# smacke/ffsubsync

Hardware: NVIDIA H100
Metric: alignments/sec (2h@100Hz signals) (higher is better)
Workload: dtype int64 VAD; f32 FFT nomination + f64 exact re-score

## Files before the change

### __graft_entry__.py

```python
import os
import subprocess
import sys

ROOT = os.path.dirname(os.path.abspath(__file__))
CSRC = os.path.join(ROOT, "ffsubsync_b200", "csrc")
LIB_DIR = os.path.join(ROOT, "ffsubsync_b200", "_lib")
LIB = os.path.join(LIB_DIR, "libffsubsync_b200.so")
EMUL = os.path.join(ROOT, "tests", "host_emul", "corr_emul")
EMUL_BIG = os.path.join(ROOT, "tests", "host_emul", "bigfft_emul")
EMUL_VAD = os.path.join(ROOT, "tests", "host_emul", "vad_emul")
EMUL_RUNS = os.path.join(ROOT, "tests", "host_emul", "runcorr_emul")

NVCC_FLAGS = [
    "-gencode", "arch=compute_90a,code=sm_90a", "-lineinfo", "-O3", "-std=c++17",
    "-Xcompiler", "-fPIC", "-Xcompiler", "-ffp-contract=off", "--fmad=true", "--extended-lambda",
    "-Wno-deprecated-gpu-targets",
]


def _sources():
    return sorted(os.path.join(CSRC, f) for f in os.listdir(CSRC) if f.endswith(".cu"))


def _stale(target, deps):
    if not os.path.exists(target):
        return True
    t = os.path.getmtime(target)
    return any(os.path.getmtime(d) > t for d in deps)


def build(force: bool = False, verbose: bool = False) -> None:
    nvcc = os.environ.get("NVCC", "/usr/local/cuda/bin/nvcc")
    os.makedirs(LIB_DIR, exist_ok=True)
    srcs = _sources()
    hdrs = [os.path.join(CSRC, f) for f in os.listdir(CSRC) if f.endswith((".cuh", ".h"))]
    hdrs.append(os.path.join(ROOT, "include", "ffsubsync_b200.h"))
    if force or _stale(LIB, srcs + hdrs):
        objs = []
        for s in srcs:
            o = os.path.join(LIB_DIR, os.path.basename(s)[:-3] + ".o")
            if force or _stale(o, [s] + hdrs):
                cmd = [nvcc] + NVCC_FLAGS + (["-Xptxas", "-v"] if verbose else []) + ["-c", s, "-o", o]
                subprocess.check_call(cmd)
            objs.append(o)
        subprocess.check_call([nvcc, "-shared", "-o", LIB] + objs + ["-Wno-deprecated-gpu-targets"])
    emu_src = EMUL + ".cu"
    if os.path.exists(emu_src) and (force or _stale(EMUL, [emu_src, os.path.join(CSRC, "corr.cuh")])):
        subprocess.check_call([nvcc, "-O2", "-std=c++17", "-Wno-deprecated-gpu-targets", "-o", EMUL, emu_src])
    big_src = EMUL_BIG + ".cu"
    if os.path.exists(big_src) and (force or _stale(EMUL_BIG, [big_src, os.path.join(CSRC, "corr.cuh"),
                                                               os.path.join(CSRC, "bigfft.cuh")])):
        subprocess.check_call([nvcc, "-O2", "-std=c++17", "--extended-lambda", "-Wno-deprecated-gpu-targets",
                               "-o", EMUL_BIG, big_src])
    runs_src = EMUL_RUNS + ".cu"
    if os.path.exists(runs_src) and (force or _stale(EMUL_RUNS, [runs_src, os.path.join(CSRC, "runcorr.cuh")])):
        subprocess.check_call([nvcc, "-O2", "-std=c++17", "-Wno-deprecated-gpu-targets", "-o", EMUL_RUNS, runs_src])
    vad_src = EMUL_VAD + ".cu"
    if os.path.exists(vad_src) and (force or _stale(EMUL_VAD, [vad_src, os.path.join(CSRC, "vad_lane.cuh"),
                                                               os.path.join(CSRC, "vad_group.cuh")])):
        subprocess.check_call([nvcc, "-O2", "-std=c++17", "-gencode", "arch=compute_90a,code=sm_90a",
                               "-Wno-deprecated-gpu-targets", "-o", EMUL_VAD, vad_src])
    sys.path.insert(0, ROOT)
    import ffsubsync_b200
    from ffsubsync_b200 import _native

    _native.load()


def smoke() -> None:
    sys.path.insert(0, ROOT)
    import numpy as np

    from ffsubsync_b200.aligners import FFTAligner, MaxScoreAligner
    from ffsubsync_b200.speech_transformers import _make_auditok_detector, _make_energy_zcr_detector
    from oracle import aligner_oracle as ao
    from oracle import auditok_oracle as au
    from oracle import vad_oracle as vo

    rng = np.random.RandomState(0)
    cls = (rng.rand(2000) > 0.5).astype(np.uint8)
    pcm = vo.synth_pcm(cls, 160, seed=1)
    got = _make_energy_zcr_detector(100, 16000, 0.0)(pcm.tobytes())
    want = vo.energy_zcr_detect(pcm.tobytes(), 100, 16000, 0.0)
    assert np.array_equal(got, want), "VAD mismatch"
    got_a = _make_auditok_detector(100, 16000, 0.0)(pcm.tobytes())
    assert np.array_equal(got_a, au.auditok_detect_fast(pcm.tobytes(), 100, 16000, 0.0)), "auditok mismatch"
    ref = want
    sub = np.concatenate([np.zeros(123), ref])[: len(ref)]
    score, off = FFTAligner(max_offset_samples=600).fit_transform(ref, sub, get_score=True)
    wscore, woff = ao.fft_align(ref, sub, 600)
    assert off == woff == -123, (off, woff)
    assert abs(score - wscore) <= 1e-5 * abs(wscore), (score, wscore)
    (s2, o2), _ = MaxScoreAligner(FFTAligner, None, 100, 6).fit_transform(ref, [sub, sub[::-1].copy()])
    assert o2 == -123
    print("smoke ok: vad windows=%d offset=%d score=%.1f" % (len(got), off, score))


if __name__ == "__main__":
    build(force="--force" in sys.argv, verbose="-v" in sys.argv)
    if "--smoke" in sys.argv:
        smoke()
```

### ffsubsync_b200/csrc/runcorr.cu

```cuda
#include <limits.h>
#include <math.h>

#include <algorithm>

#include "common.cuh"
#include "corr_jobs.cuh"
#include "runcorr.cuh"

namespace {

using namespace runcorr;
static_assert(kMaxWindow == kRunMaxWindow, "run path window bound");

struct RunRef {
  long long ref_off;
  long long q_off;
  int R;
};

struct RunStat {
  double mx;
  double eps;
  int total;
  int arg;
};

__device__ __forceinline__ int block_excl_scan(int v, int* sh, int* total) {
  const int lane = threadIdx.x & 31, warp = threadIdx.x >> 5, nw = blockDim.x >> 5;
  int x = v;
#pragma unroll
  for (int d = 1; d < 32; d <<= 1) {
    const int y = __shfl_up_sync(0xffffffffu, x, d);
    if (lane >= d) x += y;
  }
  if (lane == 31) sh[warp] = x;
  __syncthreads();
  if (warp == 0) {
    int s = lane < nw ? sh[lane] : 0;
    const int own = s;
#pragma unroll
    for (int d = 1; d < 32; d <<= 1) {
      const int y = __shfl_up_sync(0xffffffffu, s, d);
      if (lane >= d) s += y;
    }
    sh[lane] = s - own;
    if (lane == 31) sh[32] = s;
  }
  __syncthreads();
  const int r = sh[warp] + x - v;
  *total = sh[32];
  __syncthreads();
  return r;
}

__global__ void __launch_bounds__(1024) ref_bits_kernel(const float* __restrict__ ref, const RunRef* __restrict__ vids,
                                                        uint2* __restrict__ q_all) {
  __shared__ int sh[33];
  const RunRef v = vids[blockIdx.x];
  const float* r = ref + v.ref_off;
  uint2* q = q_all + v.q_off;
  const int lane = threadIdx.x & 31, warp = threadIdx.x >> 5;
  const int n_words = (v.R >> 5) + 2;
  if (threadIdx.x == 0) q[0] = make_uint2(0u, 0u);
  int carry = 0;
  for (int w0 = 0; w0 < n_words; w0 += blockDim.x) {
    const int wb = w0 + 32 * warp;
    float x[32];
#pragma unroll
    for (int u = 0; u < 32; ++u) {
      const long long i = 32LL * (wb + u) + lane;
      x[u] = i < v.R ? __ldg(r + i) : 0.f;
    }
    uint32_t mine = 0;
#pragma unroll
    for (int u = 0; u < 32; ++u) {
      const long long i = 32LL * (wb + u) + lane;
      const uint32_t bal = __ballot_sync(0xffffffffu, i < v.R && x[u] == 1.0f);
      if (lane == u) mine = bal;
    }
    const int w = wb + lane;
    int tot;
    const int ex = block_excl_scan(__popc(mine), sh, &tot);
    if (w < n_words) q[w + 1] = make_uint2(mine, (uint32_t)(carry + ex));
    carry += tot;
  }
}

__global__ void __launch_bounds__(kMaxThreads) run_corr_kernel(const SelJob* __restrict__ sel,
                                                                const long long* __restrict__ job_q,
                                                                const uint2* __restrict__ q_all,
                                                                const uint32_t* __restrict__ sub_bits,
                                                                float ref_label, int max_runs,
                                                                RunStat* __restrict__ stat,
                                                                int* __restrict__ cand_off) {
  extern __shared__ int rsm[];
  int* ra = rsm;
  int* rb = ra + max_runs;
  int* rl = rb + max_runs;
  __shared__ int sh[33];
  __shared__ double smx[32];
  __shared__ int sarg[32];
  const int j = blockIdx.x, tid = threadIdx.x, nthr = blockDim.x;
  const SelJob job = sel[j];
  if (job.kind != 0 || job.m_lo > job.m_hi) {
    if (tid == 0) stat[j] = RunStat{-INFINITY, 0.0, 0, 0};
    return;
  }
  const int R = job.R, S = job.S;
  const uint32_t* bits = sub_bits + job.bits_off;
  const int nws = S >> 5;
  int n_end = 0;
  for (int w0 = 0; w0 <= nws; w0 += nthr) {
    const int w = w0 + tid;
    uint32_t t = 0;
    if (w <= nws) {
      const int nb = S - 32 * w;
      const uint32_t x = nb >= 32 ? __ldg(bits + w) : (nb > 0 ? __ldg(bits + w) & ((1u << nb) - 1u) : 0u);
      const uint32_t prev = w > 0 ? __ldg(bits + w - 1) : 0u;
      t = x ^ ((x << 1) | (prev >> 31));
    }
    int tot;
    int idx = n_end + block_excl_scan(__popc(t), sh, &tot);
    while (t) {
      const int e = 32 * w + __ffs(t) - 1;
      t &= t - 1;
      if (idx < 2 * max_runs) (idx & 1 ? rb : ra)[idx >> 1] = e;
      ++idx;
    }
    n_end += tot;
  }
  const int nr = min(n_end >> 1, max_runs);
  __syncthreads();
  for (int r0 = 0, carry = 0; r0 < nr; r0 += nthr) {
    const int r = r0 + tid;
    const int len = r < nr ? rb[r] - ra[r] : 0;
    int tot;
    const int ex = block_excl_scan(len, sh, &tot);
    if (r < nr) rl[r] = carry + ex;
    carry += tot;
  }
  __syncthreads();
  const uint2* q = q_all + job_q[j];
  const int o_lo = job.o_first + job.m_lo, o_hi = job.o_first + job.m_hi;
  const int o0 = o_lo + kOffsetsPerThread * tid;
  const int n_mine = o0 <= o_hi ? min(kOffsetsPerThread, o_hi - o0 + 1) : 0;
  const RcLevels lv = rc_levels(job.sub_level, ref_label);
  int cnt[32], base = 0;
  if (n_mine > 0) {
    rc_thread_counts(q, R, ra, rb, nr, o0, cnt, base);
  } else {
#pragma unroll
    for (int t = 0; t < 32; ++t) cnt[t] = 0;
  }
  double best = -INFINITY;
  int barg = INT_MIN;
  {
    int um = base;
#pragma unroll
    for (int i = 0; i < 32; ++i) {
      if (i < n_mine) {
        const double g = rc_score(q, R, S, ra, rb, rl, nr, o0 + i, um, lv);
        if (g >= best) {
          best = g;
          barg = o0 + i;
        }
      }
      um += cnt[i] - nr;
    }
  }
  for (int d = 16; d > 0; d >>= 1) {
    const double ob = __shfl_xor_sync(0xffffffffu, best, d);
    const int oa = __shfl_xor_sync(0xffffffffu, barg, d);
    if (ob > best || (ob == best && oa > barg)) {
      best = ob;
      barg = oa;
    }
  }
  if ((tid & 31) == 0) {
    smx[tid >> 5] = best;
    sarg[tid >> 5] = barg;
  }
  __syncthreads();
  double mx = smx[0];
  int arg = sarg[0];
  for (int w = 1; w < (nthr >> 5); ++w)
    if (smx[w] > mx || (smx[w] == mx && sarg[w] > arg)) {
      mx = smx[w];
      arg = sarg[w];
    }
  const double eps = rc_eps((double)min(R, S), lv);
  const double cut = mx - eps;
  uint32_t hit = 0;
  {
    int um = base;
#pragma unroll
    for (int i = 0; i < 32; ++i) {
      if (i < n_mine && rc_score(q, R, S, ra, rb, rl, nr, o0 + i, um, lv) >= cut) hit |= 1u << i;
      um += cnt[i] - nr;
    }
  }
  int total;
  const int h = __popc(hit);
  int rank = block_excl_scan(h, sh, &total);
  rank = total - rank - h;
  while (hit && rank < kCandMax) {
    const int i = 31 - __clz(hit);
    hit &= ~(1u << i);
    cand_off[(size_t)j * kCandMax + rank] = o0 + i;
    ++rank;
  }
  if (tid == 0) stat[j] = RunStat{mx, eps, total, arg};
}

__global__ void __launch_bounds__(128) run_finalize_kernel(const SelJob* __restrict__ sel, int n_jobs, int K,
                                                            int winner_only, const RunStat* __restrict__ stat,
                                                            B2CandBuffers cb) {
  const int j = blockIdx.x * blockDim.x + threadIdx.x;
  if (j >= n_jobs) return;
  const SelJob job = sel[j];
  if (job.kind != 0 || job.m_lo > job.m_hi) {
    cb.cand_cnt[j] = 0;
    cb.job_stat[j] = make_float2(-INFINITY, 0.f);
    return;
  }
  const RunStat st = stat[j];
  cb.job_stat[j] = make_float2((float)st.mx, (float)st.eps);
  if (winner_only && !job.no_prune) {
    const int b0 = (j / K) * K;
    double best_floor = -INFINITY;
    for (int k = 0; k < K; ++k) {
      const RunStat s = stat[b0 + k];
      best_floor = fmax(best_floor, s.mx - s.eps);
    }
    if (fmax(st.mx, (double)(float)st.mx) + st.eps < best_floor) {
      cb.cand_off[(size_t)j * kCandMax] = st.arg;
      cb.cand_cnt[j] = -1;
      return;
    }
  }
  cb.cand_cnt[j] = st.total;
  const int n = min(st.total, kCandMax);
  const int slot = atomicAdd(cb.work_count, n);
  for (int i = 0; i < n; ++i) cb.work_list[slot + i] = (j << 5) | i;
}

}

int b2i_align_runs(b2_ctx* h, const float* d_ref, const int64_t* ref_off, int V, const int* trk_off, int K,
                   std::vector<SelJob>& sel, const uint32_t* d_bits, int max_runs, float ref_label, int winner_only,
                   const B2CandBuffers& cb, const SelJob** d_sel_out) {
  B2Range range("b2:align runs (ref_bits, run_corr, finalize)");
  const size_t J = sel.size();
  std::vector<RunRef> vids;
  std::vector<long long> job_q(J, 0);
  long long q_total = 0;
  int max_thr = 32;
  for (int v = 0; v < V; ++v) {
    const int R = (int)(ref_off[v + 1] - ref_off[v]);
    bool any = false;
    for (size_t j = (size_t)trk_off[v] * K; j < (size_t)trk_off[v + 1] * K; ++j) {
      SelJob& s = sel[j];
      if (s.kind != 0) continue;
      const long long w = (long long)s.m_hi - s.m_lo + 1;
      s.o_first = s.m_lo;
      s.m_lo = 0;
      s.m_hi = (int)(w - 1);
      max_thr = std::max<int>(max_thr, (int)(32 * ceil_div64(ceil_div64(w, kOffsetsPerThread), 32)));
      job_q[j] = q_total;
      any = true;
    }
    if (!any) continue;
    vids.push_back(RunRef{(long long)ref_off[v], q_total, R});
    q_total += rc_ref_entries(R);
  }
  if (max_thr > kMaxThreads) B2_FAIL(h, B2_ERR_UNSUPPORTED, "align runs: window wider than %d offsets", kMaxWindow);
  void* d_ws;
  const size_t q_bytes = ((size_t)q_total * 8 + 15) & ~size_t(15);
  B2_TRY(b2i_ws(h, b2_ctx::WS_RUNS, q_bytes + J * sizeof(RunStat) + 64, &d_ws));
  uint2* q = (uint2*)d_ws;
  RunStat* stat = (RunStat*)((char*)d_ws + q_bytes);
  MetaArena a;
  B2_TRY(b2i_meta_begin(h, &a, J * sizeof(SelJob) + J * 8 + vids.size() * sizeof(RunRef) + 256));
  const SelJob* d_sel = (const SelJob*)b2i_meta_put(&a, sel.data(), J * sizeof(SelJob));
  const long long* d_job_q = (const long long*)b2i_meta_put(&a, job_q.data(), J * 8);
  const RunRef* d_vids = vids.empty() ? nullptr : (const RunRef*)b2i_meta_put(&a, vids.data(), vids.size() * sizeof(RunRef));
  B2_TRY(b2i_meta_commit(&a));
  *d_sel_out = d_sel;
  if (!vids.empty()) {
    ref_bits_kernel<<<(unsigned)vids.size(), 1024, 0, h->stream>>>(d_ref, d_vids, q);
    B2_CHECK_LAUNCH(h, "ref_bits_kernel");
  }
  max_runs = std::max(1, max_runs);
  const size_t smem = (size_t)3 * max_runs * sizeof(int);
  B2_CUDA(h, cudaFuncSetAttribute(run_corr_kernel, cudaFuncAttributeMaxDynamicSharedMemorySize, (int)smem));
  run_corr_kernel<<<(unsigned)J, (unsigned)max_thr, smem, h->stream>>>(d_sel, d_job_q, q, d_bits, ref_label, max_runs,
                                                                      stat, cb.cand_off);
  B2_CHECK_LAUNCH(h, "run_corr_kernel");
  B2_CUDA(h, cudaMemsetAsync(cb.work_count, 0, sizeof(int), h->stream));
  run_finalize_kernel<<<(unsigned)((J + 127) / 128), 128, 0, h->stream>>>(d_sel, (int)J, K, winner_only, stat, cb);
  B2_CHECK_LAUNCH(h, "run_finalize_kernel");
  return B2_OK;
}
```

### ffsubsync_b200/csrc/runcorr.cuh

```cuda
#pragma once
#include <math.h>
#include <stdint.h>

#include <cuda_runtime.h>

#ifdef __CUDACC__
#define RC_HD __host__ __device__ __forceinline__
#else
#define RC_HD inline
#endif

namespace runcorr {

constexpr int kOffsetsPerThread = 32;
constexpr int kMaxThreads = 1024;
constexpr int kMaxWindow = kOffsetsPerThread * kMaxThreads;
constexpr int kRunsPerFlush = 7;

RC_HD uint32_t rc_funnel_r(uint32_t lo, uint32_t hi, int s) {
#ifdef __CUDA_ARCH__
  return __funnelshift_r(lo, hi, (unsigned)s);
#else
  return s == 0 ? lo : (lo >> s) | (hi << (32 - s));
#endif
}

RC_HD int rc_popc(uint32_t x) {
#ifdef __CUDA_ARCH__
  return __popc(x);
#else
  return __builtin_popcount(x);
#endif
}

RC_HD uint2 rc_load(const uint2* p) {
#ifdef __CUDA_ARCH__
  return __ldg(p);
#else
  return *p;
#endif
}

RC_HD long long rc_ref_entries(int R) { return (long long)(R >> 5) + 3; }

RC_HD void rc_ref_window(const uint2* q, int R, int p, uint32_t& win, int& pre) {
  p = p < -32 ? -32 : (p > R ? R : p);
  const int w = p >> 5, s = p & 31;
  const uint2 a = rc_load(q + w + 1), b = rc_load(q + w + 2);
  win = rc_funnel_r(a.x, b.x, s);
  pre = (int)a.y + rc_popc(a.x & ((1u << s) - 1u));
}

RC_HD int rc_ref_prefix(const uint2* q, int R, int p) {
  uint32_t w;
  int pre;
  rc_ref_window(q, R, p, w, pre);
  return pre;
}

RC_HD void rc_flush(uint32_t (&nib)[4], int (&cnt)[32]) {
#pragma unroll
  for (int k = 0; k < 4; ++k) {
#pragma unroll
    for (int i = 0; i < 8; ++i) cnt[4 * i + k] += (int)((nib[k] >> (4 * i)) & 15u);
    nib[k] = 0;
  }
}

RC_HD void rc_thread_counts(const uint2* q, int R, const int* ra, const int* rb, int nr, int o0, int (&cnt)[32],
                            int& base) {
#pragma unroll
  for (int t = 0; t < 32; ++t) cnt[t] = 0;
  uint32_t nib[4] = {0u, 0u, 0u, 0u};
  base = 0;
  int r = 0;
  while (r < nr) {
    const int r_end = nr - r < kRunsPerFlush ? nr : r + kRunsPerFlush;
    for (; r < r_end; ++r) {
      const int a = ra[r], b = rb[r];
      uint32_t wa, wb;
      int pa, pb;
      rc_ref_window(q, R, a + o0, wa, pa);
      rc_ref_window(q, R, b + o0, wb, pb);
      base += pb - pa;
      wa = ~wa;
#pragma unroll
      for (int k = 0; k < 4; ++k) nib[k] += ((wb >> k) & 0x11111111u) + ((wa >> k) & 0x11111111u);
    }
    rc_flush(nib, cnt);
  }
}

RC_HD int rc_sub_prefix(const int* ra, const int* rb, const int* rc, int nr, int x) {
  int lo = 0, hi = nr;
  while (lo < hi) {
    const int mid = (lo + hi) >> 1;
    if (ra[mid] < x) lo = mid + 1;
    else hi = mid;
  }
  if (lo == 0) return 0;
  const int e = rb[lo - 1] < x ? rb[lo - 1] : x;
  return rc[lo - 1] + e - ra[lo - 1];
}

struct RcLevels {
  double hi, alpha, hia;
};

RC_HD RcLevels rc_levels(float sub_level, float ref_label) {
  RcLevels l;
  l.hi = 2.0 * (double)sub_level - 1.0;
  l.alpha = 2.0 * (double)ref_label - 1.0;
  l.hia = l.hi * l.alpha;
  return l;
}

RC_HD double rc_score(const uint2* q, int R, int S, const int* ra, const int* rb, const int* rc, int nr, int o,
                      int um, const RcLevels& l) {
  const int j_lo = o < 0 ? -o : 0;
  const int j_hi = S < R - o ? S : R - o;
  if (j_hi <= j_lo) return 0.0;
  const int n_ov = j_hi - j_lo;
  const int mw = rc_ref_prefix(q, R, j_hi + o) - rc_ref_prefix(q, R, j_lo + o);
  const int uo = rc_sub_prefix(ra, rb, rc, nr, j_hi) - rc_sub_prefix(ra, rb, rc, nr, j_lo);
  const double c11 = um, c01 = mw - um, c10 = uo - um, c00 = n_ov - mw - uo + um;
  return (l.hi * c11 - c01) + (l.hia * c10 - l.alpha * c00);
}

RC_HD double rc_eps(double n, const RcLevels& l) {
  const double u = 1.1102230246251565e-16;
  const double ah = fabs(l.hi), aa = fabs(l.alpha);
  const double c = (ah > 1.0 ? ah : 1.0) * (aa > 1.0 ? aa : 1.0);
  const double k = n + 32.0;
  const double gamma = k * u / (1.0 - k * u);
  return 2.02 * (gamma + 8.0 * u) * n * c;
}

}
```

Baseline: 12460.

## Stage reference bit words in shared memory and incrementalize run-correlation scoring

Splits ref_bits_kernel into chunked blocks plus a separate prefix-fixup kernel so each video's bit-packing runs in parallel across many blocks instead of one serial block. In run_corr_kernel, reference words touched by run endpoints are staged cooperatively into shared memory spans, and per-offset counts use hierarchical nibble/byte/halfword packed accumulators. Per-offset scores now come from a precomputed window scan built with popcounts, replacing repeated binary searches and global loads. The hit pass is skipped for threads whose best score is below the cut, and a 512-thread variant with register caps is added. The cost is extra shared memory, an extra kernel launch, and more complex indexing.

```diff
diff --git a/__graft_entry__.py b/__graft_entry__.py
--- a/__graft_entry__.py
+++ b/__graft_entry__.py
@@ -10,6 +10,7 @@
 EMUL_BIG = os.path.join(ROOT, "tests", "host_emul", "bigfft_emul")
 EMUL_VAD = os.path.join(ROOT, "tests", "host_emul", "vad_emul")
 EMUL_RUNS = os.path.join(ROOT, "tests", "host_emul", "runcorr_emul")
+EMUL_STAGE = os.path.join(ROOT, "tests", "host_emul", "runcorr_stage_emul")
 
 NVCC_FLAGS = [
     "-gencode", "arch=compute_90a,code=sm_90a", "-lineinfo", "-O3", "-std=c++17",
@@ -55,6 +56,9 @@
     runs_src = EMUL_RUNS + ".cu"
     if os.path.exists(runs_src) and (force or _stale(EMUL_RUNS, [runs_src, os.path.join(CSRC, "runcorr.cuh")])):
         subprocess.check_call([nvcc, "-O2", "-std=c++17", "-Wno-deprecated-gpu-targets", "-o", EMUL_RUNS, runs_src])
+    stage_src = EMUL_STAGE + ".cu"
+    if os.path.exists(stage_src) and (force or _stale(EMUL_STAGE, [stage_src, os.path.join(CSRC, "runcorr.cuh")])):
+        subprocess.check_call([nvcc, "-O2", "-std=c++17", "-Wno-deprecated-gpu-targets", "-o", EMUL_STAGE, stage_src])
     vad_src = EMUL_VAD + ".cu"
     if os.path.exists(vad_src) and (force or _stale(EMUL_VAD, [vad_src, os.path.join(CSRC, "vad_lane.cuh"),
                                                                os.path.join(CSRC, "vad_group.cuh")])):
diff --git a/ffsubsync_b200/csrc/runcorr.cu b/ffsubsync_b200/csrc/runcorr.cu
--- a/ffsubsync_b200/csrc/runcorr.cu
+++ b/ffsubsync_b200/csrc/runcorr.cu
@@ -16,6 +16,7 @@
   long long ref_off;
   long long q_off;
   int R;
+  int tot_off;
 };
 
 struct RunStat {
@@ -25,6 +26,8 @@
   int arg;
 };
 
+constexpr int kRefChunkWords = 1024;
+
 __device__ __forceinline__ int block_excl_scan(int v, int* sh, int* total) {
   const int lane = threadIdx.x & 31, warp = threadIdx.x >> 5, nw = blockDim.x >> 5;
   int x = v;
@@ -54,49 +57,70 @@
 }
 
 __global__ void __launch_bounds__(1024) ref_bits_kernel(const float* __restrict__ ref, const RunRef* __restrict__ vids,
-                                                        uint2* __restrict__ q_all) {
+                                                        uint2* __restrict__ q_all, int* __restrict__ chunk_tot) {
   __shared__ int sh[33];
-  const RunRef v = vids[blockIdx.x];
+  const RunRef v = vids[blockIdx.y];
+  const int n_words = (v.R >> 5) + 2;
+  const int w0 = blockIdx.x * kRefChunkWords;
+  if (w0 >= n_words) return;
   const float* r = ref + v.ref_off;
   uint2* q = q_all + v.q_off;
   const int lane = threadIdx.x & 31, warp = threadIdx.x >> 5;
+  if (blockIdx.x == 0 && threadIdx.x == 0) q[0] = make_uint2(0u, 0u);
+  const int wb = w0 + 32 * warp;
+  float x[32];
+#pragma unroll
+  for (int u = 0; u < 32; ++u) {
+    const long long i = 32LL * (wb + u) + lane;
+    x[u] = i < v.R ? __ldg(r + i) : 0.f;
+  }
+  uint32_t mine = 0;
+#pragma unroll
+  for (int u = 0; u < 32; ++u) {
+    const long long i = 32LL * (wb + u) + lane;
+    const uint32_t bal = __ballot_sync(0xffffffffu, i < v.R && x[u] == 1.0f);
+    if (lane == u) mine = bal;
+  }
+  const int w = wb + lane;
+  int tot;
+  const int ex = block_excl_scan(__popc(mine), sh, &tot);
+  if (w < n_words) q[w + 1] = make_uint2(mine, (uint32_t)ex);
+  if (threadIdx.x == 0) chunk_tot[v.tot_off + blockIdx.x] = tot;
+}
+
+__global__ void __launch_bounds__(256) ref_prefix_kernel(const RunRef* __restrict__ vids, uint2* __restrict__ q_all,
+                                                         const int* __restrict__ chunk_tot) {
+  __shared__ int sh[8];
+  const RunRef v = vids[blockIdx.y];
   const int n_words = (v.R >> 5) + 2;
-  if (threadIdx.x == 0) q[0] = make_uint2(0u, 0u);
-  int carry = 0;
-  for (int w0 = 0; w0 < n_words; w0 += blockDim.x) {
-    const int wb = w0 + 32 * warp;
-    float x[32];
-#pragma unroll
-    for (int u = 0; u < 32; ++u) {
-      const long long i = 32LL * (wb + u) + lane;
-      x[u] = i < v.R ? __ldg(r + i) : 0.f;
-    }
-    uint32_t mine = 0;
-#pragma unroll
-    for (int u = 0; u < 32; ++u) {
-      const long long i = 32LL * (wb + u) + lane;
-      const uint32_t bal = __ballot_sync(0xffffffffu, i < v.R && x[u] == 1.0f);
-      if (lane == u) mine = bal;
-    }
-    const int w = wb + lane;
-    int tot;
-    const int ex = block_excl_scan(__popc(mine), sh, &tot);
-    if (w < n_words) q[w + 1] = make_uint2(mine, (uint32_t)(carry + ex));
-    carry += tot;
-  }
-}
-
-__global__ void __launch_bounds__(kMaxThreads) run_corr_kernel(const SelJob* __restrict__ sel,
-                                                                const long long* __restrict__ job_q,
-                                                                const uint2* __restrict__ q_all,
-                                                                const uint32_t* __restrict__ sub_bits,
-                                                                float ref_label, int max_runs,
-                                                                RunStat* __restrict__ stat,
-                                                                int* __restrict__ cand_off) {
+  const int c = blockIdx.x, w0 = c * kRefChunkWords;
+  if (c == 0 || w0 >= n_words) return;
+  int s = 0;
+  for (int i = threadIdx.x; i < c; i += blockDim.x) s += chunk_tot[v.tot_off + i];
+#pragma unroll
+  for (int d = 16; d > 0; d >>= 1) s += __shfl_xor_sync(0xffffffffu, s, d);
+  if ((threadIdx.x & 31) == 0) sh[threadIdx.x >> 5] = s;
+  __syncthreads();
+  s = 0;
+  for (int k = 0; k < (int)(blockDim.x >> 5); ++k) s += sh[k];
+  uint2* q = q_all + v.q_off;
+  const int w1 = min(n_words, w0 + kRefChunkWords);
+  for (int w = w0 + (int)threadIdx.x; w < w1; w += blockDim.x) q[w + 1].y += (uint32_t)s;
+}
+
+template <int kThreads>
+__global__ void __launch_bounds__(kThreads) __maxnreg__(kThreads == kSmallThreads ? 80 : 64) run_corr_kernel(const SelJob* __restrict__ sel,
+                                                             const long long* __restrict__ job_q,
+                                                             const uint2* __restrict__ q_all,
+                                                             const uint32_t* __restrict__ sub_bits,
+                                                             float ref_label, int max_runs,
+                                                             RunStat* __restrict__ stat,
+                                                             int* __restrict__ cand_off) {
   extern __shared__ int rsm[];
-  int* ra = rsm;
-  int* rb = ra + max_runs;
-  int* rl = rb + max_runs;
+  int* ends = rsm;
+  int* rl = ends + 2 * max_runs;
+  uint32_t* sb = (uint32_t*)(rl + max_runs);
+  uint32_t* sp = sb + kStageWords;
   __shared__ int sh[33];
   __shared__ double smx[32];
   __shared__ int sarg[32];
@@ -124,7 +148,7 @@
     while (t) {
       const int e = 32 * w + __ffs(t) - 1;
       t &= t - 1;
-      if (idx < 2 * max_runs) (idx & 1 ? rb : ra)[idx >> 1] = e;
+      if (idx < 2 * max_runs) ends[idx] = e;
       ++idx;
     }
     n_end += tot;
@@ -133,7 +157,7 @@
   __syncthreads();
   for (int r0 = 0, carry = 0; r0 < nr; r0 += nthr) {
     const int r = r0 + tid;
-    const int len = r < nr ? rb[r] - ra[r] : 0;
+    const int len = r < nr ? ends[2 * r + 1] - ends[2 * r] : 0;
     int tot;
     const int ex = block_excl_scan(len, sh, &tot);
     if (r < nr) rl[r] = carry + ex;
@@ -144,30 +168,42 @@
   const int o_lo = job.o_first + job.m_lo, o_hi = job.o_first + job.m_hi;
   const int o0 = o_lo + kOffsetsPerThread * tid;
   const int n_mine = o0 <= o_hi ? min(kOffsetsPerThread, o_hi - o0 + 1) : 0;
+  const RcEnds ends_k{ends};
+  RcCounts c;
+  rc_counts_init(c);
+  for (int k = 0; k < 2 * nr;) {
+    const int wlo = (ends[k] + o_lo) >> 5;
+    const int k1 = rc_span_end(ends_k, k, 2 * nr, o_lo, wlo, nthr);
+    __syncthreads();
+    for (int i = tid; i < kStageWords; i += nthr) {
+      const uint2 e = rc_ref_word(q, R, wlo + i);
+      sb[i] = e.x;
+      sp[i] = e.y;
+    }
+    __syncthreads();
+    rc_thread_span(c, sb, sp, ends_k, k, k1, o_lo, wlo, tid);
+    k = k1;
+  }
+  rc_counts_finish(c);
   const RcLevels lv = rc_levels(job.sub_level, ref_label);
-  int cnt[32], base = 0;
-  if (n_mine > 0) {
-    rc_thread_counts(q, R, ra, rb, nr, o0, cnt, base);
-  } else {
-#pragma unroll
-    for (int t = 0; t < 32; ++t) cnt[t] = 0;
-  }
   double best = -INFINITY;
   int barg = INT_MIN;
-  {
-    int um = base;
+  if (n_mine > 0) {
+    const RcScan sc = rc_scan_init(q, bits, ends_k, rl, nr, R, S, o0);
+    int um = c.base;
 #pragma unroll
     for (int i = 0; i < 32; ++i) {
       if (i < n_mine) {
-        const double g = rc_score(q, R, S, ra, rb, rl, nr, o0 + i, um, lv);
+        const double g = rc_scan_score(sc, R, S, o0, i, um, lv);
         if (g >= best) {
           best = g;
           barg = o0 + i;
         }
       }
-      um += cnt[i] - nr;
-    }
-  }
+      um += rc_count(c, i) - nr;
+    }
+  }
+  const double own = best;
   for (int d = 16; d > 0; d >>= 1) {
     const double ob = __shfl_xor_sync(0xffffffffu, best, d);
     const int oa = __shfl_xor_sync(0xffffffffu, barg, d);
@@ -191,12 +227,13 @@
   const double eps = rc_eps((double)min(R, S), lv);
   const double cut = mx - eps;
   uint32_t hit = 0;
-  {
-    int um = base;
+  if (own >= cut) {
+    const RcScan sc = rc_scan_init(q, bits, ends_k, rl, nr, R, S, o0);
+    int um = c.base;
 #pragma unroll
     for (int i = 0; i < 32; ++i) {
-      if (i < n_mine && rc_score(q, R, S, ra, rb, rl, nr, o0 + i, um, lv) >= cut) hit |= 1u << i;
-      um += cnt[i] - nr;
+      if (i < n_mine && rc_scan_score(sc, R, S, o0, i, um, lv) >= cut) hit |= 1u << i;
+      um += rc_count(c, i) - nr;
     }
   }
   int total;
@@ -254,7 +291,7 @@
   std::vector<RunRef> vids;
   std::vector<long long> job_q(J, 0);
   long long q_total = 0;
-  int max_thr = 32;
+  int max_thr = 32, n_tot = 0, max_chunks = 1;
   for (int v = 0; v < V; ++v) {
     const int R = (int)(ref_off[v + 1] - ref_off[v]);
     bool any = false;
@@ -270,15 +307,19 @@
       any = true;
     }
     if (!any) continue;
-    vids.push_back(RunRef{(long long)ref_off[v], q_total, R});
+    const int chunks = (int)ceil_div64((R >> 5) + 2, kRefChunkWords);
+    vids.push_back(RunRef{(long long)ref_off[v], q_total, R, n_tot});
     q_total += rc_ref_entries(R);
+    n_tot += chunks;
+    max_chunks = std::max(max_chunks, chunks);
   }
   if (max_thr > kMaxThreads) B2_FAIL(h, B2_ERR_UNSUPPORTED, "align runs: window wider than %d offsets", kMaxWindow);
   void* d_ws;
   const size_t q_bytes = ((size_t)q_total * 8 + 15) & ~size_t(15);
-  B2_TRY(b2i_ws(h, b2_ctx::WS_RUNS, q_bytes + J * sizeof(RunStat) + 64, &d_ws));
+  B2_TRY(b2i_ws(h, b2_ctx::WS_RUNS, q_bytes + J * sizeof(RunStat) + (size_t)n_tot * 4 + 64, &d_ws));
   uint2* q = (uint2*)d_ws;
   RunStat* stat = (RunStat*)((char*)d_ws + q_bytes);
+  int* chunk_tot = (int*)(stat + J);
   MetaArena a;
   B2_TRY(b2i_meta_begin(h, &a, J * sizeof(SelJob) + J * 8 + vids.size() * sizeof(RunRef) + 256));
   const SelJob* d_sel = (const SelJob*)b2i_meta_put(&a, sel.data(), J * sizeof(SelJob));
@@ -287,14 +328,20 @@
   B2_TRY(b2i_meta_commit(&a));
   *d_sel_out = d_sel;
   if (!vids.empty()) {
-    ref_bits_kernel<<<(unsigned)vids.size(), 1024, 0, h->stream>>>(d_ref, d_vids, q);
+    const dim3 grid((unsigned)max_chunks, (unsigned)vids.size());
+    ref_bits_kernel<<<grid, 1024, 0, h->stream>>>(d_ref, d_vids, q, chunk_tot);
     B2_CHECK_LAUNCH(h, "ref_bits_kernel");
+    if (max_chunks > 1) {
+      ref_prefix_kernel<<<grid, 256, 0, h->stream>>>(d_vids, q, chunk_tot);
+      B2_CHECK_LAUNCH(h, "ref_prefix_kernel");
+    }
   }
   max_runs = std::max(1, max_runs);
-  const size_t smem = (size_t)3 * max_runs * sizeof(int);
-  B2_CUDA(h, cudaFuncSetAttribute(run_corr_kernel, cudaFuncAttributeMaxDynamicSharedMemorySize, (int)smem));
-  run_corr_kernel<<<(unsigned)J, (unsigned)max_thr, smem, h->stream>>>(d_sel, d_job_q, q, d_bits, ref_label, max_runs,
-                                                                      stat, cb.cand_off);
+  const size_t smem = (size_t)3 * max_runs * sizeof(int) + (size_t)2 * kStageWords * sizeof(uint32_t);
+  auto kern = max_thr <= kSmallThreads ? run_corr_kernel<kSmallThreads> : run_corr_kernel<kMaxThreads>;
+  B2_CUDA(h, cudaFuncSetAttribute(kern, cudaFuncAttributeMaxDynamicSharedMemorySize, (int)smem));
+  kern<<<(unsigned)J, (unsigned)max_thr, smem, h->stream>>>(d_sel, d_job_q, q, d_bits, ref_label, max_runs, stat,
+                                                           cb.cand_off);
   B2_CHECK_LAUNCH(h, "run_corr_kernel");
   B2_CUDA(h, cudaMemsetAsync(cb.work_count, 0, sizeof(int), h->stream));
   run_finalize_kernel<<<(unsigned)((J + 127) / 128), 128, 0, h->stream>>>(d_sel, (int)J, K, winner_only, stat, cb);
diff --git a/ffsubsync_b200/csrc/runcorr.cuh b/ffsubsync_b200/csrc/runcorr.cuh
--- a/ffsubsync_b200/csrc/runcorr.cuh
+++ b/ffsubsync_b200/csrc/runcorr.cuh
@@ -10,12 +10,20 @@
 #define RC_HD inline
 #endif
 
+#ifndef RC_CHECK_INDEX
+#define RC_CHECK_INDEX(i, n) ((void)0)
+#endif
+
 namespace runcorr {
 
 constexpr int kOffsetsPerThread = 32;
 constexpr int kMaxThreads = 1024;
 constexpr int kMaxWindow = kOffsetsPerThread * kMaxThreads;
-constexpr int kRunsPerFlush = 7;
+constexpr int kSmallThreads = 512;
+constexpr int kStageWords = 2048;
+static_assert(kStageWords >= kMaxThreads + 2, "a staged span must hold one endpoint's words");
+constexpr int kEndsPerNibble = 15;
+constexpr int kNibblesPerByte = 255 / kEndsPerNibble;
 
 RC_HD uint32_t rc_funnel_r(uint32_t lo, uint32_t hi, int s) {
 #ifdef __CUDA_ARCH__
@@ -33,7 +41,8 @@
 #endif
 }
 
-RC_HD uint2 rc_load(const uint2* p) {
+template <typename T>
+RC_HD T rc_ldg(const T* p) {
 #ifdef __CUDA_ARCH__
   return __ldg(p);
 #else
@@ -43,64 +52,164 @@
 
 RC_HD long long rc_ref_entries(int R) { return (long long)(R >> 5) + 3; }
 
+RC_HD uint2 rc_ref_word(const uint2* q, int R, int g) {
+  const int last = (R >> 5) + 1;
+  g = g < -1 ? -1 : (g > last ? last : g);
+  RC_CHECK_INDEX(g + 1, rc_ref_entries(R));
+  return rc_ldg(q + g + 1);
+}
+
 RC_HD void rc_ref_window(const uint2* q, int R, int p, uint32_t& win, int& pre) {
-  p = p < -32 ? -32 : (p > R ? R : p);
   const int w = p >> 5, s = p & 31;
-  const uint2 a = rc_load(q + w + 1), b = rc_load(q + w + 2);
+  const uint2 a = rc_ref_word(q, R, w), b = rc_ref_word(q, R, w + 1);
   win = rc_funnel_r(a.x, b.x, s);
   pre = (int)a.y + rc_popc(a.x & ((1u << s) - 1u));
 }
 
-RC_HD int rc_ref_prefix(const uint2* q, int R, int p) {
-  uint32_t w;
-  int pre;
-  rc_ref_window(q, R, p, w, pre);
-  return pre;
-}
-
-RC_HD void rc_flush(uint32_t (&nib)[4], int (&cnt)[32]) {
+RC_HD uint32_t rc_sub_word(const uint32_t* bits, int S, int w) {
+  if (w < 0 || w >= ((S + 31) >> 5)) return 0u;
+  RC_CHECK_INDEX(w, (S + 31) >> 5);
+  const int nb = S - 32 * w;
+  const uint32_t x = rc_ldg(bits + w);
+  return nb >= 32 ? x : x & ((1u << nb) - 1u);
+}
+
+RC_HD uint32_t rc_sub_window(const uint32_t* bits, int S, int x) {
+  const int w = x >> 5, s = x & 31;
+  return rc_funnel_r(rc_sub_word(bits, S, w), rc_sub_word(bits, S, w + 1), s);
+}
+
+struct RcCounts {
+  uint32_t nib[4];
+  uint32_t byte[8];
+  uint32_t half[16];
+  int base;
+  int n_nib, n_byte;
+};
+
+RC_HD void rc_counts_init(RcCounts& c) {
+#pragma unroll
+  for (int k = 0; k < 4; ++k) c.nib[k] = 0u;
+#pragma unroll
+  for (int k = 0; k < 8; ++k) c.byte[k] = 0u;
+#pragma unroll
+  for (int k = 0; k < 16; ++k) c.half[k] = 0u;
+  c.base = 0;
+  c.n_nib = 0;
+  c.n_byte = 0;
+}
+
+RC_HD void rc_flush_bytes(RcCounts& c) {
+#pragma unroll
+  for (int k = 0; k < 8; ++k) {
+    c.half[k] += c.byte[k] & 0x00ff00ffu;
+    c.half[8 + k] += (c.byte[k] >> 8) & 0x00ff00ffu;
+    c.byte[k] = 0u;
+  }
+  c.n_byte = 0;
+}
+
+RC_HD int rc_count(const RcCounts& c, int t) {
+  const int i = t >> 3, k = t & 7;
+  return (int)((c.half[8 * (i & 1) + k] >> (16 * (i >> 1))) & 0xffffu);
+}
+
+RC_HD void rc_flush_nibbles(RcCounts& c) {
 #pragma unroll
   for (int k = 0; k < 4; ++k) {
-#pragma unroll
-    for (int i = 0; i < 8; ++i) cnt[4 * i + k] += (int)((nib[k] >> (4 * i)) & 15u);
-    nib[k] = 0;
-  }
-}
-
-RC_HD void rc_thread_counts(const uint2* q, int R, const int* ra, const int* rb, int nr, int o0, int (&cnt)[32],
-                            int& base) {
-#pragma unroll
-  for (int t = 0; t < 32; ++t) cnt[t] = 0;
-  uint32_t nib[4] = {0u, 0u, 0u, 0u};
-  base = 0;
-  int r = 0;
-  while (r < nr) {
-    const int r_end = nr - r < kRunsPerFlush ? nr : r + kRunsPerFlush;
-    for (; r < r_end; ++r) {
-      const int a = ra[r], b = rb[r];
-      uint32_t wa, wb;
-      int pa, pb;
-      rc_ref_window(q, R, a + o0, wa, pa);
-      rc_ref_window(q, R, b + o0, wb, pb);
-      base += pb - pa;
-      wa = ~wa;
-#pragma unroll
-      for (int k = 0; k < 4; ++k) nib[k] += ((wb >> k) & 0x11111111u) + ((wa >> k) & 0x11111111u);
+    c.byte[k] += c.nib[k] & 0x0f0f0f0fu;
+    c.byte[4 + k] += (c.nib[k] >> 4) & 0x0f0f0f0fu;
+    c.nib[k] = 0u;
+  }
+  c.n_nib = 0;
+  if (++c.n_byte == kNibblesPerByte) rc_flush_bytes(c);
+}
+
+RC_HD void rc_counts_finish(RcCounts& c) {
+  rc_flush_nibbles(c);
+  rc_flush_bytes(c);
+}
+
+RC_HD void rc_add_endpoint(RcCounts& c, int k, uint32_t lo, uint32_t hi, uint32_t pre, int s) {
+  const uint32_t flip = (uint32_t)(k & 1) - 1u;
+  const uint32_t win = rc_funnel_r(lo, hi, s) ^ flip;
+  const int m = (int)pre + rc_popc(lo & ((1u << s) - 1u));
+  c.base += (m ^ (int)flip) - (int)flip;
+#pragma unroll
+  for (int k4 = 0; k4 < 4; ++k4) c.nib[k4] += (win >> k4) & 0x11111111u;
+  if (++c.n_nib == kEndsPerNibble) rc_flush_nibbles(c);
+}
+
+struct RcEnds {
+  const int* e;
+  RC_HD int operator()(int k) const { return e[k]; }
+};
+struct RcRunArrays {
+  const int *ra, *rb;
+  RC_HD int operator()(int k) const { return (k & 1 ? rb : ra)[k >> 1]; }
+};
+
+template <typename Ends>
+RC_HD void rc_thread_span(RcCounts& c, const uint32_t* sb, const uint32_t* sp, const Ends& ends, int k0, int k1,
+                          int o_lo, int wlo, int t) {
+  for (int k = k0; k < k1; ++k) {
+    const int p = ends(k) + o_lo;
+    const int i = (p >> 5) - wlo + t;
+    RC_CHECK_INDEX(i, kStageWords);
+    RC_CHECK_INDEX(i + 1, kStageWords);
+    rc_add_endpoint(c, k, sb[i], sb[i + 1], sp[i], p & 31);
+  }
+}
+
+template <typename Ends>
+RC_HD int rc_span_end(const Ends& ends, int k0, int n, int o_lo, int wlo, int n_thr) {
+  const int lim = wlo + kStageWords - 1 - n_thr;
+  int lo = k0, hi = n;
+  while (lo < hi) {
+    const int mid = (lo + hi) >> 1;
+    if (((ends(mid) + o_lo) >> 5) <= lim) lo = mid + 1;
+    else hi = mid;
+  }
+  return lo;
+}
+
+template <typename Ends>
+inline void rc_thread_counts(const uint2* q, int R, const Ends& ends, int nr, int o0, int (&cnt)[32], int& base) {
+  RcCounts c;
+  rc_counts_init(c);
+  uint32_t sb[kStageWords], sp[kStageWords];
+  for (int k = 0; k < 2 * nr;) {
+    const int wlo = (ends(k) + o0) >> 5;
+    const int k1 = rc_span_end(ends, k, 2 * nr, o0, wlo, 1);
+    for (int i = 0; i < kStageWords; ++i) {
+      const uint2 e = rc_ref_word(q, R, wlo + i);
+      sb[i] = e.x;
+      sp[i] = e.y;
     }
-    rc_flush(nib, cnt);
-  }
-}
-
-RC_HD int rc_sub_prefix(const int* ra, const int* rb, const int* rc, int nr, int x) {
+    rc_thread_span(c, sb, sp, ends, k, k1, o0, wlo, 0);
+    k = k1;
+  }
+  rc_counts_finish(c);
+  for (int t = 0; t < 32; ++t) cnt[t] = rc_count(c, t);
+  base = c.base;
+}
+
+inline void rc_thread_counts(const uint2* q, int R, const int* ra, const int* rb, int nr, int o0, int (&cnt)[32],
+                             int& base) {
+  rc_thread_counts(q, R, RcRunArrays{ra, rb}, nr, o0, cnt, base);
+}
+
+template <typename Ends>
+RC_HD int rc_sub_prefix(const Ends& ends, const int* rl, int nr, int x) {
   int lo = 0, hi = nr;
   while (lo < hi) {
     const int mid = (lo + hi) >> 1;
-    if (ra[mid] < x) lo = mid + 1;
+    if (ends(2 * mid) < x) lo = mid + 1;
     else hi = mid;
   }
   if (lo == 0) return 0;
-  const int e = rb[lo - 1] < x ? rb[lo - 1] : x;
-  return rc[lo - 1] + e - ra[lo - 1];
+  const int e = ends(2 * lo - 1) < x ? ends(2 * lo - 1) : x;
+  return rl[lo - 1] + e - ends(2 * lo - 2);
 }
 
 struct RcLevels {
@@ -115,16 +224,53 @@
   return l;
 }
 
+RC_HD double rc_score_counts(int n_ov, int mw, int uo, int um, const RcLevels& l) {
+  const double c11 = um, c01 = mw - um, c10 = uo - um, c00 = n_ov - mw - uo + um;
+  return (l.hi * c11 - c01) + (l.hia * c10 - l.alpha * c00);
+}
+
 RC_HD double rc_score(const uint2* q, int R, int S, const int* ra, const int* rb, const int* rc, int nr, int o,
                       int um, const RcLevels& l) {
   const int j_lo = o < 0 ? -o : 0;
   const int j_hi = S < R - o ? S : R - o;
   if (j_hi <= j_lo) return 0.0;
-  const int n_ov = j_hi - j_lo;
-  const int mw = rc_ref_prefix(q, R, j_hi + o) - rc_ref_prefix(q, R, j_lo + o);
-  const int uo = rc_sub_prefix(ra, rb, rc, nr, j_hi) - rc_sub_prefix(ra, rb, rc, nr, j_lo);
-  const double c11 = um, c01 = mw - um, c10 = uo - um, c00 = n_ov - mw - uo + um;
-  return (l.hi * c11 - c01) + (l.hia * c10 - l.alpha * c00);
+  uint32_t w;
+  int m_hi, m_lo;
+  rc_ref_window(q, R, j_hi + o, w, m_hi);
+  rc_ref_window(q, R, j_lo + o, w, m_lo);
+  const RcRunArrays ends{ra, rb};
+  const int uo = rc_sub_prefix(ends, rc, nr, j_hi) - rc_sub_prefix(ends, rc, nr, j_lo);
+  return rc_score_counts(j_hi - j_lo, m_hi - m_lo, uo, um, l);
+}
+
+struct RcScan {
+  uint32_t wm_lo, wm_hi;
+  uint32_t wu_lo, wu_hi;
+  int m_lo, m_hi, u_lo, u_hi;
+};
+
+template <typename Ends>
+RC_HD RcScan rc_scan_init(const uint2* q, const uint32_t* bits, const Ends& ends, const int* rl, int nr, int R,
+                          int S, int o0) {
+  RcScan sc;
+  rc_ref_window(q, R, o0, sc.wm_lo, sc.m_lo);
+  rc_ref_window(q, R, S + o0, sc.wm_hi, sc.m_hi);
+  sc.wu_lo = rc_sub_window(bits, S, -o0 - 31);
+  sc.wu_hi = rc_sub_window(bits, S, R - o0 - 31);
+  sc.u_lo = rc_sub_prefix(ends, rl, nr, -o0 - 31);
+  sc.u_hi = rc_sub_prefix(ends, rl, nr, R - o0 - 31);
+  return sc;
+}
+
+RC_HD double rc_scan_score(const RcScan& sc, int R, int S, int o0, int i, int um, const RcLevels& l) {
+  const int o = o0 + i;
+  const int j_lo = o < 0 ? -o : 0;
+  const int j_hi = S < R - o ? S : R - o;
+  if (j_hi <= j_lo) return 0.0;
+  const uint32_t below_i = (1u << i) - 1u, below_ui = 0x7fffffffu >> i;
+  const int mw = (sc.m_hi + rc_popc(sc.wm_hi & below_i)) - (sc.m_lo + rc_popc(sc.wm_lo & below_i));
+  const int uo = (sc.u_hi + rc_popc(sc.wu_hi & below_ui)) - (sc.u_lo + rc_popc(sc.wu_lo & below_ui));
+  return rc_score_counts(j_hi - j_lo, mw, uo, um, l);
 }
 
 RC_HD double rc_eps(double n, const RcLevels& l) {
```

Result: no change. 12440, median of 6 (-0.1%).
